# google-research/hyperbo

Hardware: AMD Instinct MI355X
Metric: GP NLL+grad evals/sec at N=8192 D=16 fp64 (higher is better)
Workload: dtype f64

## Files before the change

hyperbo_amd/csrc/chol.hip:

```cpp
#include "hbo_internal.h"
#include <type_traits>
#include <limits.h>
#include <string.h>

namespace {

#include "panel_dev.h"
#ifdef HBO_POTF2_TIMING
__device__ unsigned long long hbo_dbg_stamps[64];
__device__ unsigned long long hbo_dbg_wall[3 * 256];
__device__ unsigned long long hbo_dbg_trsm[3 * 128];
__device__ int hbo_dbg_trsm_panel = 36;
#define STAMP(i) do { if (threadIdx.x == 0) hbo_dbg_stamps[i] = __builtin_readcyclecounter(); } while (0)
#else
#define STAMP(i) do {} while (0)
#endif
#ifndef HBO_POTF2_WAVES
#define HBO_POTF2_WAVES 8
#endif
constexpr int POTF2_WAVES = HBO_POTF2_WAVES;
constexpr int POTF2_THREADS = 64 * POTF2_WAVES;
template <typename T>
__device__ __forceinline__ void potf2_body(const TaskDesc& t, int p, int* info_slot, unsigned char* smem) {
  typedef typename Mma<T>::acc_t acc_t;
  T* sT = reinterpret_cast<T*>(smem);
  T* sM = sT + 36 * TILE_ELEMS;
  T* sDinv = sM + TILE_ELEMS;
  const int64_t ld = t.ld;
  T* Ab = static_cast<T*>(t.A) + (int64_t)p * NB * ld + (int64_t)p * NB;
  T* Wb = static_cast<T*>(t.W) + (int64_t)p * NB * ld + (int64_t)p * NB;
  const int tid = threadIdx.x, lane = tid & 63, wave = tid >> 6;
  const int l15 = lane & 15, lq = lane >> 4;
  const int ei = (tid & 255) >> 4, ej = tid & 15;
  STAMP(0);
#ifdef HBO_POTF2_TIMING
  if (tid == 0 && blockIdx.x == 0 && p < 256) {
    hbo_dbg_wall[3 * p] = wall_clock64();
    hbo_dbg_wall[3 * p + 2] = ((unsigned long long)__builtin_amdgcn_s_getreg((20 << 0) | (0 << 6) | (31 << 11)) << 32) |
                              (unsigned)__builtin_amdgcn_s_getreg((4 << 0) | (0 << 6) | (31 << 11));
  }
#endif

  auto factor_leaf = [&](int jb, const acc_t* from_regs = nullptr) {
    T* dt = sT + tri_index(jb, jb) * TILE_ELEMS;
    acc_t acc;
    if (from_regs) acc = *from_regs;
    else {
#pragma unroll
      for (int r = 0; r < 4; ++r) acc[r] = dt[Mma<T>::crow(lane, r) * TS + l15];
    }
    const int bad = leaf_cholesky4<T>(acc, dt, sM, sDinv + jb * 16, Wb + (int64_t)(jb * 16) * ld + jb * 16, ld, lane);
    if (bad >= 0 && lane == 0) atomicMin(info_slot, p * NB + jb * 16 + bad + 1);
  };
  auto solve_tile = [&](int jb, int R) {
    T* xt = sT + tri_index(R, jb) * TILE_ELEMS;
    acc_t acc = {0, 0, 0, 0};
#pragma unroll
    for (int kk = 0; kk < 4; ++kk) acc = Mma<T>::mma(xt[l15 * TS + kk * 4 + lq], sM[l15 * TS + kk * 4 + lq], acc);
#pragma unroll
    for (int r = 0; r < 4; ++r) xt[Mma<T>::crow(lane, r) * TS + l15] = acc[r];
  };
  auto update_tile = [&](int jb, int I, int J) {
    T* ct = sT + tri_index(I, J) * TILE_ELEMS;
    const T* at = sT + tri_index(I, jb) * TILE_ELEMS;
    const T* bt = sT + tri_index(J, jb) * TILE_ELEMS;
    acc_t acc;
#pragma unroll
    for (int r = 0; r < 4; ++r) acc[r] = ct[Mma<T>::crow(lane, r) * TS + l15];
#pragma unroll
    for (int kk = 0; kk < 4; ++kk) acc = Mma<T>::mma(-at[l15 * TS + kk * 4 + lq], bt[l15 * TS + kk * 4 + lq], acc);
#pragma unroll
    for (int r = 0; r < 4; ++r) ct[Mma<T>::crow(lane, r) * TS + l15] = acc[r];
  };

  auto update_tile2 = [&](int jb, int I0, int J0, int I1, int J1) {
    T* c0 = sT + tri_index(I0, J0) * TILE_ELEMS;
    T* c1 = sT + tri_index(I1, J1) * TILE_ELEMS;
    const T* a0 = sT + tri_index(I0, jb) * TILE_ELEMS;
    const T* b0 = sT + tri_index(J0, jb) * TILE_ELEMS;
    const T* a1 = sT + tri_index(I1, jb) * TILE_ELEMS;
    const T* b1 = sT + tri_index(J1, jb) * TILE_ELEMS;
    acc_t x0, x1;
    T fa0[4], fb0[4], fa1[4], fb1[4];
#pragma unroll
    for (int r = 0; r < 4; ++r) { x0[r] = c0[Mma<T>::crow(lane, r) * TS + l15]; x1[r] = c1[Mma<T>::crow(lane, r) * TS + l15]; }
#pragma unroll
    for (int kk = 0; kk < 4; ++kk) {
      fa0[kk] = -a0[l15 * TS + kk * 4 + lq]; fb0[kk] = b0[l15 * TS + kk * 4 + lq];
      fa1[kk] = -a1[l15 * TS + kk * 4 + lq]; fb1[kk] = b1[l15 * TS + kk * 4 + lq];
    }
#pragma unroll
    for (int kk = 0; kk < 4; ++kk) { x0 = Mma<T>::mma(fa0[kk], fb0[kk], x0); x1 = Mma<T>::mma(fa1[kk], fb1[kk], x1); }
#pragma unroll
    for (int r = 0; r < 4; ++r) { c0[Mma<T>::crow(lane, r) * TS + l15] = x0[r]; c1[Mma<T>::crow(lane, r) * TS + l15] = x1[r]; }
  };

  int nleaf = 8;
  {
    const int64_t rows = (int64_t)t.n - (int64_t)p * NB;
    if (rows < NB) nleaf = rows <= 0 ? 0 : (int)((rows + 15) / 16);
    for (int jb = nleaf + wave; jb < 8; jb += POTF2_WAVES)
#pragma unroll
      for (int r = 0; r < 4; ++r) {
        const int row = Mma<T>::crow(lane, r);
        gst(Wb + (int64_t)(jb * 16 + row) * ld + jb * 16 + l15, row == l15 ? (T)1 : (T)0);
      }
    if (tid < NB && tid >= nleaf * 16) sDinv[tid] = (T)1;
  }
  const bool lead_tile0 = nleaf > 0;
  acc_t tile0 = {0, 0, 0, 0};
  if (wave == 0 && lead_tile0) {
#pragma unroll
    for (int r = 0; r < 4; ++r) {
      const int row = Mma<T>::crow(lane, r);
      const int rr = row > l15 ? row : l15, cc = row > l15 ? l15 : row;
      tile0[r] = gld(Ab + (int64_t)rr * ld + cc);
    }
  }
  constexpr int NSH = POTF2_THREADS / 256;
  const int sh = __builtin_amdgcn_readfirstlane(tid >> 8);
  T vload[36 / NSH];
  auto load_issue = [&](auto share) {
    constexpr int SH = decltype(share)::value;
    int tile = 0;
#pragma unroll
    for (int I = 0; I < 8; ++I)
#pragma unroll
      for (int J = 0; J <= I; ++J, ++tile) {
        if (tile % NSH != SH) continue;
        if (tile == 0 && lead_tile0) { vload[0] = (T)0; continue; }
        int r = ei, c = ej;
        if (I == J && ej > ei) { r = ej; c = ei; }
        vload[tile / NSH] = gld(Ab + (int64_t)(I * 16 + r) * ld + J * 16 + c);
      }
  };
  auto load_commit = [&](auto share) {
    constexpr int SH = decltype(share)::value;
#pragma unroll
    for (int k = 0; k < 36 / NSH; ++k)
      if (!(k == 0 && SH == 0 && lead_tile0)) sT[(k * NSH + SH) * TILE_ELEMS + ei * TS + ej] = vload[k];
  };
  static_assert(NSH == 1 || NSH == 2, "one or two 256-thread groups");
  if (NSH == 1 || sh == 0) load_issue(std::integral_constant<int, 0>());
  else load_issue(std::integral_constant<int, NSH - 1>());
  if (wave == 0 && lead_tile0) factor_leaf(0, &tile0);
  if (NSH == 1 || sh == 0) load_commit(std::integral_constant<int, 0>());
  else load_commit(std::integral_constant<int, NSH - 1>());
  STAMP(1);
  __syncthreads();
  STAMP(2);
  for (int jb = 0; jb < nleaf; ++jb) {
    for (int R = jb + 1 + wave; R < nleaf; R += POTF2_WAVES) solve_tile(jb, R);
    __syncthreads();
    STAMP(3 + 3 * jb);
    if (jb == nleaf - 1) break;
    {
      const int m = nleaf - 1 - jb;
      const int ntiles = m * (m + 1) / 2;
      constexpr int NH = POTF2_WAVES == 8 ? 6 : POTF2_WAVES - 1;
      const int hw = POTF2_WAVES == 8 ? (wave < 4 ? wave : wave - 1) : wave;
      const int n0 = (ntiles - 1 > 4 * NH + 1) ? (ntiles - 1 - (4 * NH + 1)) / POTF2_WAVES : 0;
      const int nshared = ntiles - n0;
      auto tile_of = [&](int tix, int& I, int& J) {
        int ii = 0;
        while ((ii + 1) * (ii + 2) / 2 <= tix) ++ii;
        I = jb + 1 + ii; J = jb + 1 + tix - ii * (ii + 1) / 2;
      };
      if (wave == 0) {
        update_tile(jb, jb + 1, jb + 1);
        factor_leaf(jb + 1);
        STAMP(4 + 3 * jb);
        for (int tix = nshared; tix < ntiles; ++tix) { int I, J; tile_of(tix, I, J); update_tile(jb, I, J); }
      } else if (!(POTF2_WAVES == 8 && wave == 4)) {
        int tix = hw;
        for (; tix + NH < nshared; tix += 2 * NH) {
          int I0, J0, I1, J1;
          tile_of(tix, I0, J0); tile_of(tix + NH, I1, J1);
          update_tile2(jb, I0, J0, I1, J1);
        }
        if (tix < nshared) { int I, J; tile_of(tix, I, J); update_tile(jb, I, J); }
      }
    }
    __syncthreads();
    STAMP(5 + 3 * jb);
  }
  STAMP(30);

  auto store_share = [&](auto share) {
    constexpr int SH = decltype(share)::value;
    int tile = 0;
#pragma unroll
    for (int I = 0; I < 8; ++I)
#pragma unroll
      for (int J = 0; J <= I; ++J, ++tile) {
        if (tile % NSH != SH) continue;
        T v = sT[tile * TILE_ELEMS + ei * TS + ej];
        if (I == J && ej > ei) v = (T)0;
        gst(Ab + (int64_t)(I * 16 + ei) * ld + J * 16 + ej, v);
      }
  };
  if (NSH == 1 || sh == 0) store_share(std::integral_constant<int, 0>());
  else store_share(std::integral_constant<int, NSH - 1>());
  STAMP(31);
  STAMP(32);
#ifdef HBO_POTF2_TIMING
  if (tid == 0 && blockIdx.x == 0 && p < 256) hbo_dbg_wall[3 * p + 1] = wall_clock64();
#endif
}
template <typename T>
__global__ __launch_bounds__(POTF2_THREADS) void potf2_kernel(const TaskDesc* tasks, int p, int* info, int* yield_flag, unsigned long long* tl) {
  extern __shared__ __attribute__((aligned(16))) unsigned char smem[];
  __builtin_amdgcn_s_setprio(3);
  const TaskDesc& t = tasks[blockIdx.x];
  if (p >= t.nblk) return;
  tl_begin(tl);
  int tok = 0;
  if (yield_flag && threadIdx.x == 0) tok = yield_enter(yield_flag);
  potf2_body<T>(t, p, info + blockIdx.x, smem);
  if (yield_flag) {
    __syncthreads();
    if (threadIdx.x == 0) yield_leave(yield_flag, tok);
  }
  tl_end(tl);
}

template <typename T>
constexpr int trsm_tile() { return sizeof(T) == 8 ? 256 : TILE_ELEMS; }
template <typename T>
__device__ __forceinline__ int trsm_at(int r, int c) { return sizeof(T) == 8 ? r * 16 + (c ^ ((r >> 1) << 1)) : r * TS + c; }
template <typename T>
constexpr int trsm_lds_bytes() { return (28 + 8 + 4) * trsm_tile<T>() * (int)sizeof(T); }
__device__ __forceinline__ int strict_index(int I, int J) { return I * (I - 1) / 2 + J; }

template <typename T, bool IDENT>
__device__ __forceinline__ void trsm_body(const TaskDesc& t, int p, int64_t row0, unsigned char* smem, bool stage,
                                          unsigned short* xp = nullptr, int nkb = 0, int kb_off = 0) {
  typedef typename Mma<T>::acc_t acc_t;
  constexpr int TE = trsm_tile<T>();
  T* sLt = reinterpret_cast<T*>(smem);
  T* sWi = sLt + 28 * TE;
  T* sSc = sWi + 8 * TE;
  const int64_t ld = t.ld;
  const int tid = threadIdx.x, lane = tid & 63, wave = tid >> 6;
  const int l15 = lane & 15, lq = lane >> 4;
  const T* Lb = static_cast<const T*>(t.A) + (int64_t)p * NB * ld + (int64_t)p * NB;
  const T* Wb = static_cast<const T*>(t.W) + (int64_t)p * NB * ld + (int64_t)p * NB;

  const int64_t wrow0 = row0 + wave * 16;
  const int rg = IDENT ? (int)((wrow0 - (int64_t)p * NB) >> 4) : 0;
  T* Ap = IDENT ? nullptr : static_cast<T*>(t.A) + wrow0 * ld + (int64_t)p * NB;
  T* Wout = IDENT ? static_cast<T*>(t.W) + (int64_t)p * NB * ld + (int64_t)p * NB : nullptr;

  acc_t areg[8];
#pragma unroll
  for (int jb = 0; jb < 8; ++jb)
#pragma unroll
    for (int r = 0; r < 4; ++r) {
      const int row = Mma<T>::crow(lane, r);
      if (IDENT) areg[jb][r] = (rg == jb && row == l15) ? (T)1 : (T)0;
      else areg[jb][r] = gld(Ap + (int64_t)row * ld + jb * 16 + l15);
    }
  if (stage) {
    const int i = tid >> 4, j = tid & 15;
    int tile = 0;
#pragma unroll
    for (int I = 1; I < 8; ++I)
#pragma unroll
      for (int J = 0; J < I; ++J, ++tile)
        sLt[tile * TE + trsm_at<T>(i, j)] = gld(Lb + (int64_t)(I * 16 + i) * ld + J * 16 + j);
#pragma unroll
    for (int b = 0; b < 8; ++b)
      sWi[b * TE + trsm_at<T>(i, j)] = gld(Wb + (int64_t)(b * 16 + i) * ld + b * 16 + j);
  }
  if (stage) __syncthreads();

  T* sc = sSc + wave * TE;
  T xneg[8][4];
#pragma unroll
  for (int jb = 0; jb < 8; ++jb) {
    acc_t acc = areg[jb];
    acc_t acc2 = (acc_t){0, 0, 0, 0};
#pragma unroll
    for (int kb = 0; kb < 8; ++kb) {
      if (kb < jb) {
        const T* lt = sLt + strict_index(jb, kb) * TE;
#pragma unroll
        for (int kk = 0; kk < 4; ++kk) {
          const T bfrag = lt[trsm_at<T>(l15, kk * 4 + lq)];
          if (kb & 1) acc2 = Mma<T>::mma(xneg[kb][kk], bfrag, acc2);
          else acc = Mma<T>::mma(xneg[kb][kk], bfrag, acc);
        }
      }
    }
#pragma unroll
    for (int r = 0; r < 4; ++r) acc[r] += acc2[r];
    __builtin_amdgcn_wave_barrier();
#pragma unroll
    for (int r = 0; r < 4; ++r) sc[trsm_at<T>(Mma<T>::crow(lane, r), l15)] = acc[r];
    __builtin_amdgcn_wave_barrier();
    T ta[4];
#pragma unroll
    for (int kk = 0; kk < 4; ++kk) ta[kk] = sc[trsm_at<T>(l15, kk * 4 + lq)];
    acc_t x = (acc_t){0, 0, 0, 0};
    const T* wt = sWi + jb * TE;
#pragma unroll
    for (int kk = 0; kk < 4; ++kk) {
      const T bfrag = wt[trsm_at<T>(l15, kk * 4 + lq)];
      x = Mma<T>::mma(ta[kk], bfrag, x);
    }
#pragma unroll
    for (int r = 0; r < 4; ++r) {
      const int row = Mma<T>::crow(lane, r);
      if (IDENT) {
        if (rg != jb) gst(Wout + (int64_t)(jb * 16 + l15) * ld + rg * 16 + row, x[r]);
      } else {
        gst(Ap + (int64_t)row * ld + jb * 16 + l15, x[r]);
        if constexpr (sizeof(T) == 4) {
          if (xp) {
            const int64_t grow = wrow0 + row;
            unsigned short h, m, l;
            hbo_split3((float)x[r], h, m, l);
            unsigned short* o = xp + ((grow / NB * nkb + kb_off + jb) * 3) * (int64_t)(NB * 16) + (grow % NB) * 16 + l15;
            o[0] = h; o[NB * 16] = m; o[2 * NB * 16] = l;
          }
        }
      }
    }
    if (jb < 7) {
      __builtin_amdgcn_wave_barrier();
#pragma unroll
      for (int r = 0; r < 4; ++r) sc[trsm_at<T>(Mma<T>::crow(lane, r), l15)] = x[r];
      __builtin_amdgcn_wave_barrier();
#pragma unroll
      for (int kk = 0; kk < 4; ++kk) xneg[jb][kk] = -sc[trsm_at<T>(l15, kk * 4 + lq)];
    }
  }
}
template <typename T, bool IDENT>
__global__ __launch_bounds__(256) void trsm_kernel(const TaskDesc* tasks, int p_arg, int* yield_tab, SplitOut so, unsigned long long* tl) {
  extern __shared__ __attribute__((aligned(16))) unsigned char smem[];
  __builtin_amdgcn_s_setprio(3);
  const TaskDesc& t = tasks[blockIdx.z];
  const int p = IDENT ? p_arg + (int)blockIdx.y : p_arg;
  if (p >= t.nblk) return;
#ifdef HBO_POTF2_TIMING
  const bool dbg = !IDENT && p == hbo_dbg_trsm_panel && blockIdx.x < 128 && threadIdx.x == 0;
  if (dbg) {
    hbo_dbg_trsm[3 * blockIdx.x] = wall_clock64();
    hbo_dbg_trsm[3 * blockIdx.x + 2] = ((unsigned long long)__builtin_amdgcn_s_getreg((20 << 0) | (0 << 6) | (31 << 11)) << 32) |
                                       (unsigned)__builtin_amdgcn_s_getreg((4 << 0) | (0 << 6) | (31 << 11));
  }
#endif
  int64_t row0;
  if (IDENT) {
    row0 = (int64_t)p * NB + (int64_t)blockIdx.x * 64;
  } else {
    const int64_t first = (int64_t)(p + 1) * NB;
    const int64_t nrows = (int64_t)(t.nblk + 1) * NB - first;
    const int64_t bx = ((int64_t)blockIdx.x + 3 * (int64_t)blockIdx.z) % gridDim.x;
    if (bx * 64 >= nrows) return;
    row0 = first + bx * 64;
  }
  int tok = 0;
  tl_begin(tl);
  if (yield_tab && threadIdx.x == 0) tok = yield_enter(yield_tab);
  trsm_body<T, IDENT>(t, p, row0, smem, true, so.xp ? so.xp + (int64_t)blockIdx.z * so.task_stride : nullptr, so.nkb, so.kb_off);
  if (yield_tab) {
    __syncthreads();
    if (threadIdx.x == 0) yield_leave(yield_tab, tok);
  }
  tl_end(tl);
#ifdef HBO_POTF2_TIMING
  if (dbg) hbo_dbg_trsm[3 * blockIdx.x + 1] = wall_clock64();
#endif
}

#ifndef HBO_DEVICE_ONLY
template <typename T>
void set_attrs() {
  static unsigned long long seen = 0;
  if (!hbo_first_use_on_device(seen)) return;
  hipFuncSetAttribute(reinterpret_cast<const void*>(&potf2_kernel<T>),
                      hipFuncAttributeMaxDynamicSharedMemorySize, potf2_lds_bytes<T>());
  hipFuncSetAttribute(reinterpret_cast<const void*>(&trsm_kernel<T, false>),
                      hipFuncAttributeMaxDynamicSharedMemorySize, trsm_lds_bytes<T>());
  hipFuncSetAttribute(reinterpret_cast<const void*>(&trsm_kernel<T, true>),
                      hipFuncAttributeMaxDynamicSharedMemorySize, trsm_lds_bytes<T>());
}

template <typename T>
void potf2_t(const TaskDesc* tasks, int ntasks, int p, int* info, hipStream_t st, int* yield_flag, unsigned long long* tl) {
  set_attrs<T>();
  hipLaunchKernelGGL((potf2_kernel<T>), dim3(ntasks), dim3(POTF2_THREADS), potf2_lds_bytes<T>(), st, tasks, p, info,
                     yield_flag, tl);
}
template <typename T>
void trsm_t(const TaskDesc* tasks, int ntasks, int p, int max_nblk, hipStream_t st, int* yield_tab, const SplitOut& so, unsigned long long* tl) {
  set_attrs<T>();
  const int nrows = (max_nblk + 1 - (p + 1)) * NB;
  if (nrows <= 0) return;
  hipLaunchKernelGGL((trsm_kernel<T, false>), dim3(nrows / 64, 1, ntasks), dim3(256), trsm_lds_bytes<T>(), st,
                     tasks, p, yield_tab, so, tl);
}
template <typename T>
void trtri_diag_t(const TaskDesc* tasks, int ntasks, int p_lo, int p_hi, hipStream_t st) {
  set_attrs<T>();
  if (p_hi <= p_lo) return;
  SplitOut none; memset(&none, 0, sizeof none);
  hipLaunchKernelGGL((trsm_kernel<T, true>), dim3(2, p_hi - p_lo, ntasks), dim3(256), trsm_lds_bytes<T>(), st,
                     tasks, p_lo, (int*)nullptr, none, (unsigned long long*)nullptr);
}

#endif
}

#ifndef HBO_DEVICE_ONLY
#ifdef HBO_POTF2_TIMING
void dbg_read_stamps(unsigned long long* host) { hipMemcpyFromSymbol(host, HIP_SYMBOL(hbo_dbg_stamps), sizeof(unsigned long long) * 64); }
extern "C" void hbo_dbg_trsm_wall(unsigned long long* host, int panel) {
  if (host) hipMemcpyFromSymbol(host, HIP_SYMBOL(hbo_dbg_trsm), sizeof(unsigned long long) * 3 * 128);
  else hipMemcpyToSymbol(HIP_SYMBOL(hbo_dbg_trsm_panel), &panel, sizeof(int));
}
extern "C" void hbo_dbg_potf2_wall(unsigned long long* host) { hipMemcpyFromSymbol(host, HIP_SYMBOL(hbo_dbg_wall), sizeof(unsigned long long) * 3 * 256); }
#endif
void launch_potf2(int dtype, const TaskDesc* tasks, int ntasks, int p, int* info, hipStream_t st, int* yield_flag, unsigned long long* tl) {
  if (dtype == HBO_F64) potf2_t<double>(tasks, ntasks, p, info, st, yield_flag, tl);
  else potf2_t<float>(tasks, ntasks, p, info, st, yield_flag, tl);
}
void launch_trsm(int dtype, const TaskDesc* tasks, int ntasks, int p, int max_nblk, hipStream_t st, int* yield_tab, const SplitOut* so,
                 unsigned long long* tl) {
  SplitOut o; memset(&o, 0, sizeof o);
  if (so) o = *so;
  if (dtype == HBO_F64) trsm_t<double>(tasks, ntasks, p, max_nblk, st, yield_tab, o, tl);
  else trsm_t<float>(tasks, ntasks, p, max_nblk, st, yield_tab, o, tl);
}
void launch_trtri_diag(int dtype, const TaskDesc* tasks, int ntasks, int p_lo, int p_hi, hipStream_t st) {
  if (dtype == HBO_F64) trtri_diag_t<double>(tasks, ntasks, p_lo, p_hi, st);
  else trtri_diag_t<float>(tasks, ntasks, p_lo, p_hi, st);
}
#endif
```

hyperbo_amd/csrc/panel_dev.h:

```cpp
#pragma once

template <typename T> struct Mma;
template <> struct Mma<double> {
  typedef double acc_t __attribute__((ext_vector_type(4)));
  static __device__ __forceinline__ acc_t mma(double a, double b, acc_t c) {
    return __builtin_amdgcn_mfma_f64_16x16x4f64(a, b, c, 0, 0, 0);
  }
  static __device__ __forceinline__ int crow(int lane, int r) { return (lane >> 4) + 4 * r; }
};
template <> struct Mma<float> {
  typedef float acc_t __attribute__((ext_vector_type(4)));
  static __device__ __forceinline__ acc_t mma(float a, float b, acc_t c) {
    return __builtin_amdgcn_mfma_f32_16x16x4f32(a, b, c, 0, 0, 0);
  }
  static __device__ __forceinline__ int crow(int lane, int r) { return 4 * (lane >> 4) + r; }
};

constexpr int NB = HBO_TILE;

__device__ __forceinline__ double readlane_t(double v, int lane) {
  int lo = __double2loint(v), hi = __double2hiint(v);
  lo = __builtin_amdgcn_readlane(lo, lane);
  hi = __builtin_amdgcn_readlane(hi, lane);
  return __hiloint2double(hi, lo);
}
__device__ __forceinline__ double swap16(double v) {
  int lo = __double2loint(v), hi = __double2hiint(v);
  lo = __builtin_amdgcn_ds_swizzle(lo, 0x401F);
  hi = __builtin_amdgcn_ds_swizzle(hi, 0x401F);
  return __hiloint2double(hi, lo);
}
__device__ __forceinline__ float swap16(float v) {
  return __int_as_float(__builtin_amdgcn_ds_swizzle(__float_as_int(v), 0x401F));
}
__device__ __forceinline__ float readlane_t(float v, int lane) {
  return __int_as_float(__builtin_amdgcn_readlane(__float_as_int(v), lane));
}
__device__ __forceinline__ double lane_gather(double v, int src) {
  int lo = __double2loint(v), hi = __double2hiint(v);
  lo = __builtin_amdgcn_ds_bpermute(src << 2, lo);
  hi = __builtin_amdgcn_ds_bpermute(src << 2, hi);
  return __hiloint2double(hi, lo);
}
__device__ __forceinline__ float lane_gather(float v, int src) {
  return __int_as_float(__builtin_amdgcn_ds_bpermute(src << 2, __float_as_int(v)));
}

constexpr int TS = 17;
constexpr int TILE_ELEMS = 16 * TS;
__device__ __forceinline__ int tri_index(int I, int J) { return I * (I + 1) / 2 + J; }


template <typename T>
constexpr int potf2_lds_bytes() { return (37 * TILE_ELEMS + NB) * (int)sizeof(T); }

__device__ __forceinline__ double fast_rsqrt(double d) {
  const double y = __builtin_amdgcn_rsq(d);
  const double e = fma(-d * y, y, 1.0);
  return fma(y * e, fma(e, 0.375, 0.5), y);
}
__device__ __forceinline__ float fast_rsqrt(float d) { return rsqrt(d); }

template <typename T>
__device__ __forceinline__ int leaf_cholesky4(typename Mma<T>::acc_t& acc, T* dt, T* sM, T* dinv_out, T* Wg, int64_t ldw, int lane) {
  typedef typename Mma<T>::acc_t acc_t;
  constexpr bool F64 = sizeof(T) == 8;
  const int l15 = lane & 15, lq = lane >> 4;
  acc_t vinv;
#pragma unroll
  for (int r = 0; r < 4; ++r) vinv[r] = (Mma<T>::crow(lane, r) == l15) ? (T)1 : (T)0;
#pragma unroll
  for (int j = 0; j < 16; j += 4) {
    const int g0 = j >> 2;
    T s[4], v[4];
    T p00, p10, p11, p20, p21, p22, p30, p31, p32, p33;
    if constexpr (F64) {
      const T own = acc[g0], vown = vinv[g0];
      p00 = readlane_t(own, j);
      p10 = readlane_t(own, 16 + j); p11 = readlane_t(own, 16 + j + 1);
      p20 = readlane_t(own, 32 + j); p21 = readlane_t(own, 32 + j + 1); p22 = readlane_t(own, 32 + j + 2);
      p30 = readlane_t(own, 48 + j); p31 = readlane_t(own, 48 + j + 1); p32 = readlane_t(own, 48 + j + 2); p33 = readlane_t(own, 48 + j + 3);
#pragma unroll
      for (int a = 0; a < 4; ++a) { s[a] = lane_gather(own, 16 * a + l15); v[a] = lane_gather(vown, 16 * a + l15); }
    } else {
      const int base = 16 * g0;
      p00 = readlane_t(acc[0], base + j);
      p10 = readlane_t(acc[1], base + j); p11 = readlane_t(acc[1], base + j + 1);
      p20 = readlane_t(acc[2], base + j); p21 = readlane_t(acc[2], base + j + 1); p22 = readlane_t(acc[2], base + j + 2);
      p30 = readlane_t(acc[3], base + j); p31 = readlane_t(acc[3], base + j + 1); p32 = readlane_t(acc[3], base + j + 2); p33 = readlane_t(acc[3], base + j + 3);
#pragma unroll
      for (int a = 0; a < 4; ++a) { s[a] = lane_gather(acc[a], base + l15); v[a] = lane_gather(vinv[a], base + l15); }
    }
    auto inv_sqrt = [](T d) -> T {
      if constexpr (F64) return fast_rsqrt(d);
      else return d > (T)0 ? fast_rsqrt(d) : (T)NAN;
    };
    const T i0 = inv_sqrt(p00);
    const T l10 = p10 * i0, l20 = p20 * i0, l30 = p30 * i0;
    const T i1 = inv_sqrt(fma(-l10, l10, p11));
    const T l21 = fma(-l20, l10, p21) * i1, l31 = fma(-l30, l10, p31) * i1;
    const T i2 = inv_sqrt(fma(-l21, l21, fma(-l20, l20, p22)));
    const T l32 = fma(-l31, l21, fma(-l30, l20, p32)) * i2;
    const T i3 = inv_sqrt(fma(-l32, l32, fma(-l31, l31, fma(-l30, l30, p33))));
    dinv_out[j] = i0; dinv_out[j + 1] = i1; dinv_out[j + 2] = i2; dinv_out[j + 3] = i3;
    const T f0 = s[0] * i0;
    const T f1 = fma(-l10, f0, s[1]) * i1;
    const T f2 = fma(-l21, f1, fma(-l20, f0, s[2])) * i2;
    const T f3 = fma(-l32, f2, fma(-l31, f1, fma(-l30, f0, s[3]))) * i3;
    const T a = (lq == 0) ? f0 : (lq == 1 ? f1 : (lq == 2 ? f2 : f3));
    acc = Mma<T>::mma(-a, a, acc);
    __builtin_amdgcn_sched_barrier(0);
    const T h0 = v[0] * i0;
    const T h1 = fma(-l10, h0, v[1]) * i1;
    const T h2 = fma(-l21, h1, fma(-l20, h0, v[2])) * i2;
    const T h3 = fma(-l32, h2, fma(-l31, h1, fma(-l30, h0, v[3]))) * i3;
    const T b = (lq == 0) ? h0 : (lq == 1 ? h1 : (lq == 2 ? h2 : h3));
    vinv = Mma<T>::mma(-a, b, vinv);
    dt[l15 * TS + j + lq] = a;
    sM[(j + lq) * TS + l15] = b;
    gst(Wg + (int64_t)(j + lq) * ldw + l15, b);
    __builtin_amdgcn_sched_barrier(0);
  }
  const T mine = dinv_out[l15];
  const unsigned long long badmask = __ballot(!(mine < (T)INFINITY)) & 0xFFFFull;
  return badmask ? (int)__builtin_ctzll(badmask) : -1;
}
```

Measured before the change: 85.95.

## Overlap panel column stores with trailing updates and use permlane row broadcasts

```diff
diff --git a/hyperbo_amd/csrc/chol.hip b/hyperbo_amd/csrc/chol.hip
--- a/hyperbo_amd/csrc/chol.hip
+++ b/hyperbo_amd/csrc/chol.hip
@@ -149,11 +149,25 @@
   STAMP(1);
   __syncthreads();
   STAMP(2);
+  constexpr int STORE_WAVE = POTF2_WAVES == 8 ? 4 : POTF2_WAVES - 1;
+  auto store_col = [&](int jb) {
+    for (int I = jb; I < 8; ++I) {
+      const T* tt = sT + tri_index(I, jb) * TILE_ELEMS;
+#pragma unroll
+      for (int r = 0; r < 4; ++r) {
+        const int row = 4 * r + lq;
+        T v = tt[row * TS + l15];
+        if (I == jb && l15 > row) v = (T)0;
+        gst(Ab + (int64_t)(I * 16 + row) * ld + jb * 16 + l15, v);
+      }
+    }
+  };
   for (int jb = 0; jb < nleaf; ++jb) {
     for (int R = jb + 1 + wave; R < nleaf; R += POTF2_WAVES) solve_tile(jb, R);
     __syncthreads();
     STAMP(3 + 3 * jb);
     if (jb == nleaf - 1) break;
+    if (wave == STORE_WAVE) store_col(jb);
     {
       const int m = nleaf - 1 - jb;
       const int ntiles = m * (m + 1) / 2;
@@ -186,21 +200,7 @@
   }
   STAMP(30);
 
-  auto store_share = [&](auto share) {
-    constexpr int SH = decltype(share)::value;
-    int tile = 0;
-#pragma unroll
-    for (int I = 0; I < 8; ++I)
-#pragma unroll
-      for (int J = 0; J <= I; ++J, ++tile) {
-        if (tile % NSH != SH) continue;
-        T v = sT[tile * TILE_ELEMS + ei * TS + ej];
-        if (I == J && ej > ei) v = (T)0;
-        gst(Ab + (int64_t)(I * 16 + ei) * ld + J * 16 + ej, v);
-      }
-  };
-  if (NSH == 1 || sh == 0) store_share(std::integral_constant<int, 0>());
-  else store_share(std::integral_constant<int, NSH - 1>());
+  for (int jb = (nleaf > 0 ? nleaf - 1 : 0) + wave; jb < 8; jb += POTF2_WAVES) store_col(jb);
   STAMP(31);
   STAMP(32);
 #ifdef HBO_POTF2_TIMING
diff --git a/hyperbo_amd/csrc/panel_dev.h b/hyperbo_amd/csrc/panel_dev.h
--- a/hyperbo_amd/csrc/panel_dev.h
+++ b/hyperbo_amd/csrc/panel_dev.h
@@ -24,26 +24,28 @@
   hi = __builtin_amdgcn_readlane(hi, lane);
   return __hiloint2double(hi, lo);
 }
-__device__ __forceinline__ double swap16(double v) {
-  int lo = __double2loint(v), hi = __double2hiint(v);
-  lo = __builtin_amdgcn_ds_swizzle(lo, 0x401F);
-  hi = __builtin_amdgcn_ds_swizzle(hi, 0x401F);
-  return __hiloint2double(hi, lo);
-}
-__device__ __forceinline__ float swap16(float v) {
-  return __int_as_float(__builtin_amdgcn_ds_swizzle(__float_as_int(v), 0x401F));
-}
 __device__ __forceinline__ float readlane_t(float v, int lane) {
   return __int_as_float(__builtin_amdgcn_readlane(__float_as_int(v), lane));
 }
-__device__ __forceinline__ double lane_gather(double v, int src) {
-  int lo = __double2loint(v), hi = __double2hiint(v);
-  lo = __builtin_amdgcn_ds_bpermute(src << 2, lo);
-  hi = __builtin_amdgcn_ds_bpermute(src << 2, hi);
-  return __hiloint2double(hi, lo);
+__device__ __forceinline__ void row_bcast4(unsigned v, unsigned out[4]) {
+  const auto p = __builtin_amdgcn_permlane16_swap(v, v, false, false);
+  const auto e = __builtin_amdgcn_permlane32_swap(p[0], p[0], false, false);
+  const auto o = __builtin_amdgcn_permlane32_swap(p[1], p[1], false, false);
+  out[0] = e[0]; out[1] = o[0]; out[2] = e[1]; out[3] = o[1];
 }
-__device__ __forceinline__ float lane_gather(float v, int src) {
-  return __int_as_float(__builtin_amdgcn_ds_bpermute(src << 2, __float_as_int(v)));
+__device__ __forceinline__ void row_bcast4(double v, double out[4]) {
+  unsigned lo[4], hi[4];
+  row_bcast4((unsigned)__double2loint(v), lo);
+  row_bcast4((unsigned)__double2hiint(v), hi);
+#pragma unroll
+  for (int a = 0; a < 4; ++a) out[a] = __hiloint2double((int)hi[a], (int)lo[a]);
+}
+__device__ __forceinline__ float row_bcast(float v, int g) {
+  const unsigned u = __float_as_uint(v);
+  const auto p = __builtin_amdgcn_permlane16_swap(u, u, false, false);
+  const unsigned h = (g & 1) ? p[1] : p[0];
+  const auto e = __builtin_amdgcn_permlane32_swap(h, h, false, false);
+  return __uint_as_float((g & 2) ? e[1] : e[0]);
 }
 
 constexpr int TS = 17;
@@ -75,13 +77,12 @@
     T s[4], v[4];
     T p00, p10, p11, p20, p21, p22, p30, p31, p32, p33;
     if constexpr (F64) {
-      const T own = acc[g0], vown = vinv[g0];
+      const T own = acc[g0];
       p00 = readlane_t(own, j);
       p10 = readlane_t(own, 16 + j); p11 = readlane_t(own, 16 + j + 1);
       p20 = readlane_t(own, 32 + j); p21 = readlane_t(own, 32 + j + 1); p22 = readlane_t(own, 32 + j + 2);
       p30 = readlane_t(own, 48 + j); p31 = readlane_t(own, 48 + j + 1); p32 = readlane_t(own, 48 + j + 2); p33 = readlane_t(own, 48 + j + 3);
-#pragma unroll
-      for (int a = 0; a < 4; ++a) { s[a] = lane_gather(own, 16 * a + l15); v[a] = lane_gather(vown, 16 * a + l15); }
+      row_bcast4(own, s);
     } else {
       const int base = 16 * g0;
       p00 = readlane_t(acc[0], base + j);
@@ -89,7 +90,7 @@
       p20 = readlane_t(acc[2], base + j); p21 = readlane_t(acc[2], base + j + 1); p22 = readlane_t(acc[2], base + j + 2);
       p30 = readlane_t(acc[3], base + j); p31 = readlane_t(acc[3], base + j + 1); p32 = readlane_t(acc[3], base + j + 2); p33 = readlane_t(acc[3], base + j + 3);
 #pragma unroll
-      for (int a = 0; a < 4; ++a) { s[a] = lane_gather(acc[a], base + l15); v[a] = lane_gather(vinv[a], base + l15); }
+      for (int a = 0; a < 4; ++a) s[a] = row_bcast(acc[a], g0);
     }
     auto inv_sqrt = [](T d) -> T {
       if constexpr (F64) return fast_rsqrt(d);
@@ -110,6 +111,11 @@
     const T a = (lq == 0) ? f0 : (lq == 1 ? f1 : (lq == 2 ? f2 : f3));
     acc = Mma<T>::mma(-a, a, acc);
     __builtin_amdgcn_sched_barrier(0);
+    if constexpr (F64) row_bcast4(vinv[g0], v);
+    else {
+#pragma unroll
+      for (int a = 0; a < 4; ++a) v[a] = row_bcast(vinv[a], g0);
+    }
     const T h0 = v[0] * i0;
     const T h1 = fma(-l10, h0, v[1]) * i1;
     const T h2 = fma(-l21, h1, fma(-l20, h0, v[2])) * i2;
```

Result: no change. 85.98, median of 6 (+0.0%).
